# deepomicslab/PALACE

Hardware: AMD Instinct MI355X
Metric: contigs/sec eref+generate_graph+matching, 1M-contig synth, 1/2/4/8 GPU (higher is better)
Workload: dtype u32

## Files before the change

palace_amd/csrc/eref.hip:

```cpp
#include "eref_common.hpp"

namespace palace {

__global__ __launch_bounds__(256) void eref_count_kernel(const uint8_t *__restrict__ bases,
                                                         const int64_t *__restrict__ offsets,
                                                         int64_t n_reads,
                                                         const uint8_t *__restrict__ keep,
                                                         CoderMasks masks, KeyBuckets range, uint32_t *__restrict__ p1,
                                                         uint32_t *__restrict__ p2,
                                                         uint32_t *__restrict__ p3)
{
    const int lane = threadIdx.x & 63;
    const int64_t wave = (static_cast<int64_t>(blockIdx.x) * blockDim.x + threadIdx.x) >> 6;
    const int64_t n_waves = (static_cast<int64_t>(gridDim.x) * blockDim.x) >> 6;
    for (int64_t r = wave; r < n_reads; r += n_waves) {
        if (keep && !keep[r]) continue;
        const int64_t beg = offsets[r];
        const int64_t len = offsets[r + 1] - beg;
        const int64_t npos = len - 31;
        if (npos <= 0) continue;
        const uint8_t *s = bases + beg;
        Streams lo = ballot_streams(s, lane, len);
        for (int64_t base = 0; base < npos; base += 64) {
            Streams hi = ballot_streams(s, base + 64 + lane, len);
// ... 196 lines not shown
                  "the 6-position tile must fit four times into the LDS of a CU");
    __shared__ uint32_t dst[kL1Buckets];
    __shared__ uint32_t any_partial;
    const int lane = threadIdx.x & 63, wave = threadIdx.x >> 6;
#ifdef PALACE_STAMPS
    unsigned long long stamp_arr[8] = {0, 0, 0, 0, 0, 0, 0, 0};
    unsigned long long *stamps = (threadIdx.x == 0 && blockIdx.x % 7 == 0 && blockIdx.x / 7 < 65536) ? stamp_arr : nullptr;
#endif
    STAMP(stamps, 0);
    const int64_t p = pos_lo + (static_cast<int64_t>(blockIdx.x) * THREADS + threadIdx.x) * P;
    const int64_t g = min(p, pos_hi) >> 5;
    const int sh = static_cast<int>(p & 31);
    uint32_t w[2][3], uw[2];
#pragma unroll
    for (int q = 0; q < 3; q++) { w[0][q] = s0[g + q]; w[1][q] = s1[g + q]; }
    uw[0] = su[g]; uw[1] = su[g + 1];
    if (threadIdx.x < kL1Buckets) hist[threadIdx.x] = 0;
    if (threadIdx.x == kL1Buckets) any_partial = 0;
    lds_barrier();
    uint32_t u = __builtin_amdgcn_alignbit(uw[1], uw[0], sh) & ((1u << P) - 1);
    if (p >= pos_hi) u = 0;
    else if (p + P > pos_hi) u &= (1u << (pos_hi - p)) - 1;
    uint32_t key[P][3], rank[P][3];
    if (u) {
        uint32_t lo[2], hi[2];
#pragma unroll
        for (int q = 0; q < 2; q++) {
            lo[q] = __builtin_amdgcn_alignbit(w[q][1], w[q][0], sh);
            hi[q] = __builtin_amdgcn_alignbit(w[q][2], w[q][1], sh);
        }
#pragma unroll
        for (int t = 0; t < P; t++) {
            const uint32_t a0 = __builtin_amdgcn_alignbit(hi[0], lo[0], t), a1 = __builtin_amdgcn_alignbit(hi[1], lo[1], t);
            kmer_keys(masks, a0, a1, ~(a0 ^ a1), key[t]);
            if ((u >> t) & 1u) {
#pragma unroll
                for (int i = 0; i < 3; i++) {
                    const uint32_t bk = key[t][i] >> kL1Shift;
                    rank[t][i] = (!SHARE || o.keys.bucket(bk)) ? atomicAdd(&hist[bk], 1u) : ~0u;
                }
            }
        }
    }
    STAMP(stamps, 1);
    lds_barrier();
    STAMP(stamps, 2);
    const uint32_t replica = blockIdx.x % kL1Replicas;
    const bool reserver = threadIdx.x >= 64 && threadIdx.x < 64 + kL1Buckets;
    const uint32_t my_row = threadIdx.x - 64;
    uint32_t my_pc = 0, my_g = 0;
    if (wave == 0) {
        const uint32_t c0 = hist[2 * lane], c1 = hist[2 * lane + 1];
        const uint32_t pc0 = (c0 + kGroupKeys - 1) / kGroupKeys * kGroupKeys, pc1 = (c1 + kGroupKeys - 1) / kGroupKeys * kGroupKeys;
        const uint32_t incl = wave_inclusive_scan(pc0 + pc1);
        const uint32_t a0 = incl - pc0 - pc1, a1 = a0 + pc0;
        start[2 * lane] = a0; start[2 * lane + 1] = a1;
        if (lane == 63) start[kL1Buckets] = incl;
    } else if (reserver) {
        my_pc = (hist[my_row] + kGroupKeys - 1) / kGroupKeys;
        if (my_pc) my_g = atomicAdd(&o.cursor[l1_cursor(my_row, replica)], my_pc);
    }
    lds_barrier();
    STAMP(stamps, 3);
    if (u) {
#pragma unroll
        for (int t = 0; t < P; t++) {
            if ((u >> t) & 1u) {
#pragma unroll
                for (int i = 0; i < 3; i++)
                    if (!SHARE || rank[t][i] != ~0u) tile[start[key[t][i] >> kL1Shift] + rank[t][i]] = key[t][i];
            }
        }
    }
    if (reserver) {
        const uint32_t cap = o.caps.cap(my_row);
        const bool whole = static_cast<uint64_t>(my_g) + my_pc <= cap;
        room[my_row] = cap - min(cap, my_g);
        dst[my_row] = static_cast<uint32_t>(l1_region_base(o.caps, my_row, replica) + my_g - start[my_row] / kGroupKeys);
        if (!whole) any_partial = 1;
    }
    lds_barrier();
    STAMP(stamps, 4);
    const uint32_t total = start[kL1Buckets];
    const bool check = any_partial != 0;
    constexpr int kSweeps = (kMaxKeys / static_cast<int>(kGroupKeys) + THREADS - 1) / THREADS;
    uint32_t slow = 0;
    uint4 k[kSweeps];
    uint32_t to[kSweeps], live = 0;
#pragma unroll
    for (int it = 0; it < kSweeps; it++) {
        const uint32_t gi = it * THREADS + threadIdx.x, x = gi * kGroupKeys;
        to[it] = 0;
        k[it] = uint4{0, 0, 0, 0};
        if (x < total) {
            uint32_t s5[kGroupKeys];
#pragma unroll
            for (uint32_t e = 0; e < kGroupKeys; e++) s5[e] = tile[x + e];
            const uint32_t row = s5[0] >> kL1Shift;
            const uint32_t in_row = x - start[row];
            k[it] = pack_group(s5, min(kGroupKeys, hist[row] - in_row));
            if (!check || in_row / kGroupKeys < room[row]) { to[it] = dst[row] + gi; live |= 1u << it; }
            else slow |= 1u << it;
        }
    }
#pragma unroll
    for (int it = 0; it < kSweeps; it++)
        if (live & (1u << it)) reinterpret_cast<uint4 *>(o.buf)[to[it]] = k[it];
    if (slow) {
#pragma unroll 1
        for (int it = 0; it < kSweeps; it++) {
            if (!((slow >> it) & 1u)) continue;
            const uint32_t x = (it * THREADS + threadIdx.x) * kGroupKeys;
            const uint32_t row = tile[x] >> kL1Shift;
            const uint32_t n = min(kGroupKeys, hist[row] - (x - start[row]));
#pragma unroll 1
            for (uint32_t e = 0; e < n; e++) count_key_marked(tile[x + e], o.p1, o.p2, o.p3, o.touched);
        }
    }
    STAMP(stamps, 5);
#ifdef PALACE_STAMPS
    asm volatile("s_waitcnt vmcnt(0)" ::: "memory");
    STAMP(stamps, 6);
    if (stamps)
        for (int i = 0; i < 8; i++) palace_stamp_buf[(blockIdx.x / 7) * 8 + i] = stamp_arr[i];
#endif
}

__global__ __launch_bounds__(kBin2Threads) void eref_bin2_kernel(const unsigned int *__restrict__ cursor1,
                                                                 const uint32_t *__restrict__ buf1, DensityCaps caps1,
                                                                 Bin2Grid grid, Bin2Out o)
{
    __shared__ Stage2 st;
    uint32_t lo = 0, hi = kL1Buckets;
    while (hi - lo > 1) { const uint32_t mid = (lo + hi) >> 1; if (grid.first[mid] <= blockIdx.x) lo = mid; else hi = mid; }
    const uint32_t b1 = lo, within = blockIdx.x - grid.first[b1], per_region = tiles_of_bucket(caps1, b1);
    const uint32_t replica = within / per_region, tile = within % per_region;
    const uint32_t n1 = min(cursor1[l1_cursor(b1, replica)], caps1.cap(b1));
    const uint32_t start = tile * kTile2Groups;
    if (start >= n1) return;
    const uint32_t end = min(n1, start + kTile2Groups);
    const uint4 *src = reinterpret_cast<const uint4 *>(buf1) + l1_region_base(caps1, b1, replica);
    uint4 v[kGroups2PerThread];
#pragma unroll
    for (int it = 0; it < kGroups2PerThread; it++) {
        const uint32_t i = start + it * kBin2Threads + threadIdx.x;
        v[it] = i < end ? src[i] : uint4{0, 0, 0, 0};
    }
    if (threadIdx.x < kL2Rows) st.rows[threadIdx.x] = threadIdx.x * kRowSlots;
    const uint32_t cap = fine_sub_cap(o.caps, b1), xcd = xcc_id();
    __syncthreads();
    using Homeless = std::conditional_t<(kGroups2PerThread * kGroupKeys > 32), unsigned long long, uint32_t>;
    Homeless homeless = 0;
#pragma unroll
    for (int it = 0; it < kGroups2PerThread; it++) {
        uint32_t k[kGroupKeys];
        const uint32_t n = unpack_group(v[it], k);
        uint32_t at[kGroupKeys];
#pragma unroll
        for (uint32_t e = 0; e < kGroupKeys; e++) at[e] = atomicAdd(&st.rows[k[e] >> kFineBits], e < n ? 1u : 0u);
#pragma unroll
        for (uint32_t e = 0; e < kGroupKeys; e++) {
            const uint32_t row = k[e] >> kFineBits;
            const bool is_key = e < n, fits = at[e] < (row + 1) * kRowSlots;
            st.slot[is_key && fits ? at[e] : kStage2Slots] = static_cast<uint16_t>(k[e]);
            homeless |= static_cast<Homeless>(is_key && !fits ? 1u : 0u) << (kGroupKeys * it + e);
        }
    }
    if (homeless) {
#pragma unroll
        for (int it = 0; it < kGroups2PerThread; it++) {
            if (!((homeless >> (kGroupKeys * it)) & 31u)) continue;
            uint32_t k[kGroupKeys];
            unpack_group(src[start + it * kBin2Threads + threadIdx.x], k);
#pragma unroll
            for (uint32_t e = 0; e < kGroupKeys; e++) {
                if (!((homeless >> (kGroupKeys * it + e)) & 1u)) continue;
                const uint32_t row = k[e] >> kFineBits;
                const uint32_t gg = atomicAdd(&o.cursor[(b1 * kL2Rows + row) * kXcds + xcd], 1u);
                if (gg < cap) o.buf[fine_region_base(o.caps, b1, row) + static_cast<uint64_t>(xcd) * cap + gg] = static_cast<uint16_t>(k[e]);
                else count_key_marked((b1 << kL1Shift) | k[e], o.p1, o.p2, o.p3, o.touched);
            }
        }
    }
    __syncthreads();
    constexpr int rows_per_wave = kL2Rows / (kBin2Threads / 64);
    const int lane = threadIdx.x & 63;
    const int row0 = __builtin_amdgcn_readfirstlane(static_cast<int>(threadIdx.x >> 6)) * rows_per_wave;
    uint32_t c = 0, g = 0, p_lo = 0, p_hi = 0;
    bool over = false;
    if (lane < rows_per_wave) {
        const uint32_t row = row0 + lane;
        c = min(st.rows[row], (row + 1) * kRowSlots) - row * kRowSlots;
        if (c) g = atomicAdd(&o.cursor[(b1 * kL2Rows + row) * kXcds + xcd], c);
        over = static_cast<uint64_t>(g) + c > cap;
        const uint64_t ptr = reinterpret_cast<uint64_t>(o.buf + fine_region_base(o.caps, b1, row) + static_cast<uint64_t>(xcd) * cap + min(g, cap));
        p_lo = static_cast<uint32_t>(ptr); p_hi = static_cast<uint32_t>(ptr >> 32);
    }
    const unsigned long long over_rows = __ballot(over);
    const uint32_t c_fast = over ? 0u : c;
#pragma unroll
    for (int j0 = 0; j0 < rows_per_wave; j0 += 16) {
        uint16_t k[16];
#pragma unroll
        for (int j = 0; j < 16; j++) k[j] = st.slot[(row0 + j0 + j) * kRowSlots + lane];
#pragma unroll
        for (int j = 0; j < 16; j++) {
            const uint32_t cj = __builtin_amdgcn_readlane(c_fast, j0 + j);
            const uint32_t bl = __builtin_amdgcn_readlane(p_lo, j0 + j), bh = __builtin_amdgcn_readlane(p_hi, j0 + j);
            global_u16 *dst = reinterpret_cast<global_u16 *>((static_cast<uint64_t>(bh) << 32) | bl);
            if (lane < cj) dst[lane] = k[j];
        }
    }
    unsigned long long more = __ballot(lane < rows_per_wave && (c > 64 || over));
    while (more) {
        const int j = __builtin_ctzll(more);
        more &= more - 1;
        const uint32_t cj = __builtin_amdgcn_readlane(c, j);
        const uint32_t bl = __builtin_amdgcn_readlane(p_lo, j), bh = __builtin_amdgcn_readlane(p_hi, j);
        global_u16 *dst = reinterpret_cast<global_u16 *>((static_cast<uint64_t>(bh) << 32) | bl);
        const uint16_t *row_slots = st.slot + (row0 + j) * kRowSlots;
        if ((over_rows >> j) & 1ull) {
            const uint32_t gj = __builtin_amdgcn_readlane(g, j);
            const uint32_t room = cap - (gj < cap ? gj : cap);
            const uint32_t fine = b1 * kL2Rows + row0 + j;
#pragma unroll 1
            for (uint32_t q = 0; q < cj; q += 64) {
                if (q + lane < cj) {
                    const uint32_t kk = row_slots[q + lane];
                    if (q + lane < room) dst[q + lane] = static_cast<uint16_t>(kk);
                    else count_key_marked((fine << kFineBits) | kk, o.p1, o.p2, o.p3, o.touched);
                }
            }
            continue;
        }
        for (uint32_t q = 64; q < cj; q += 64)
            if (lane + q < cj) dst[lane + q] = row_slots[lane + q];
    }
}

constexpr int kCountThreads = 256;
constexpr int kProbeSetsMax = 4;
struct ProbeArgs {
    const unsigned long long *first[kProbeSetsMax];
    const uint16_t *keys16[kProbeSetsMax];
    uint8_t *ehits[kProbeSetsMax];
    const uint32_t *pos_s;
    uint8_t *sent_bytes;
};
__device__ __forceinline__ void scatter_sentinels(const ProbeArgs &pr, unsigned long long i, uint32_t m)
{
    uint32_t p[8];
#pragma unroll
    for (int e = 0; e < 8; e++) p[e] = ((m >> e) & 1u) ? pr.pos_s[i * 8 + e] : ~0u;
#pragma unroll
    for (int e = 0; e < 8; e++)
        if (p[e] != ~0u) pr.sent_bytes[p[e]] = 1;
}
__device__ __forceinline__ uint32_t count_vector(const uint32_t *__restrict__ l1, const uint32_t *__restrict__ l2, const uint32_t *__restrict__ l3, const uint4 &v)
{
    const uint32_t d[4] = {v.x, v.y, v.z, v.w};
    uint32_t m = 0;
#pragma unroll
    for (int e = 0; e < 4; e++) {
        const uint32_t k0 = d[e] & 0xffffu, k1 = d[e] >> 16;
        const uint32_t c0 = ((l1[k0 >> 5] >> (k0 & 31)) & 1u) + ((l2[k0 >> 5] >> (k0 & 31)) & 1u) + ((l3[k0 >> 5] >> (k0 & 31)) & 1u);
        const uint32_t c1 = ((l1[k1 >> 5] >> (k1 & 31)) & 1u) + ((l2[k1 >> 5] >> (k1 & 31)) & 1u) + ((l3[k1 >> 5] >> (k1 & 31)) & 1u);
        m |= c0 << (4 * e);
        m |= c1 << (4 * e + 2);
    }
    return m;
}

template <bool CLEAN, bool FINAL = false, int PROBE = 0>
__global__ __launch_bounds__(kCountThreads) void eref_lds_count_kernel(const unsigned int *__restrict__ cursor,
                                                                       const uint16_t *__restrict__ binned,
                                                                       DensityCaps caps, uint32_t *__restrict__ p1,
                                                                       uint32_t *__restrict__ p2,
                                                                       uint32_t *__restrict__ p3,
                                                                       const unsigned int *__restrict__ touched, KeyBuckets share,
                                                                       ProbeArgs pr)
{
    __shared__ uint32_t l1[kFineWords], l2[kFineWords], l3[kFineWords];
    const uint32_t b = blockIdx.x, b1 = b / kL2Rows;
    if (!share.bucket(b1)) return;
    constexpr int kProbeBatch = 2;
    unsigned long long pe0 = 0, phi = 0;
    if (PROBE) { pe0 = pr.first[0][b] / 8; phi = pr.first[0][b + 1] / 8; }
    constexpr int kLateCh = 3, kLateSent = 1;
#ifndef PALACE_PROBE_GROUP
#define PALACE_PROBE_GROUP 2
#endif
    constexpr int kProbeGroup = PALACE_PROBE_GROUP;
    constexpr bool ALL = PROBE >= 2, COUNTS = PROBE == 3;
    auto code = [&](const uint4 &vec) -> uint32_t { return COUNTS ? count_vector(l1, l2, l3, vec) : probe_vector(l3, vec); };
    auto put_code = [&](int k, unsigned long long i, uint32_t m) {
        if (COUNTS) reinterpret_cast<uint16_t *>(pr.ehits[k])[i] = static_cast<uint16_t>(m);
        else pr.ehits[k][i] = static_cast<uint8_t>(m);
    };
    unsigned long long q0[kProbeSetsMax - 1] = {0, 0, 0}, q1[kProbeSetsMax - 1] = {0, 0, 0};
    if (ALL) {
#pragma unroll
        for (int k = 1; k < kProbeSetsMax; k++) { q0[k - 1] = pr.first[k][b] / 8; q1[k - 1] = pr.first[k][b + 1] / 8; }
    }
    const uint32_t sub_cap = fine_sub_cap(caps, b1);
    uint32_t n_sub[kXcds], first[kXcds + 1];
    first[0] = 0;
#pragma unroll
    for (int x = 0; x < kXcds; x++) {
        n_sub[x] = min(cursor[b * kXcds + x], sub_cap);
        first[x + 1] = first[x] + (n_sub[x] + 7) / 8;
    }
    const uint32_t n8 = first[kXcds];
    const size_t w0 = static_cast<size_t>(b) * kFineWords;
    if (n8 == 0) {
        if (FINAL && ((touched[b >> 5] >> (b & 31)) & 1u)) {
            uint4 *z1 = reinterpret_cast<uint4 *>(p1 + w0), *z2 = reinterpret_cast<uint4 *>(p2 + w0);
            if (COUNTS) {
                for (int i = threadIdx.x; i < kFineWords / 4; i += kCountThreads) {
                    reinterpret_cast<uint4 *>(l1)[i] = z1[i];
                    reinterpret_cast<uint4 *>(l2)[i] = z2[i];
                }
            }
            for (int i = threadIdx.x; i < kFineWords / 4; i += kCountThreads) z1[i] = z2[i] = uint4{0, 0, 0, 0};
            if (ALL || (PROBE && phi > pe0)) {
                const uint4 *s3 = reinterpret_cast<const uint4 *>(p3 + w0);
                for (int i = threadIdx.x; i < kFineWords / 4; i += kCountThreads) reinterpret_cast<uint4 *>(l3)[i] = s3[i];
                __syncthreads();
                const uint4 *pv = reinterpret_cast<const uint4 *>(pr.keys16[0]);
                for (unsigned long long i = pe0 + threadIdx.x; i < phi; i += kCountThreads) put_code(0, i, code(pv[i]));
                if (ALL) {
#pragma unroll
                    for (int k = 1; k < kProbeSetsMax; k++) {
                        const uint4 *qv = reinterpret_cast<const uint4 *>(pr.keys16[k]);
                        for (unsigned long long i = q0[k - 1] + threadIdx.x; i < q1[k - 1]; i += kCountThreads) {
                            const uint32_t m = code(qv[i]);
                            if (k == 3 && !COUNTS) scatter_sentinels(pr, i, m);
                            else put_code(k, i, m);
                        }
                    }
                    uint4 *z3 = reinterpret_cast<uint4 *>(p3 + w0);
                    for (int i = threadIdx.x; i < kFineWords / 4; i += kCountThreads) z3[i] = uint4{0, 0, 0, 0};
                }
            }
        }
        return;
    }
    const uint4 *g1 = reinterpret_cast<const uint4 *>(p1 + w0), *g2 = reinterpret_cast<const uint4 *>(p2 + w0),
                *g3 = reinterpret_cast<const uint4 *>(p3 + w0);
    const uint4 *keys = reinterpret_cast<const uint4 *>(binned + fine_region_base(caps, b1, b % kL2Rows));
    auto locate = [&](uint32_t j, uint32_t &valid) -> const uint4 * {
        uint32_t x = 0, f = 0, ns = n_sub[0];
#pragma unroll
        for (int k = 1; k < kXcds; k++) {
            const uint32_t ge = j >= first[k] ? 1u : 0u;
            x += ge; f += ge * (first[k] - first[k - 1]); ns += ge * (n_sub[k] - n_sub[k - 1]);
        }
        const uint32_t local = j - f;
        valid = min(8u, ns - 8 * local);
        return keys + (static_cast<size_t>(x) * sub_cap) / 8 + local;
    };
    constexpr int kBatch = 4;
    uint4 v[kBatch];
    uint32_t ok[kBatch];
#pragma unroll
    for (int u = 0; u < kBatch; u++) {
        const uint32_t i = threadIdx.x + u * kCountThreads;
        ok[u] = 0; v[u] = uint4{0, 0, 0, 0};
        if (i < n8) v[u] = *locate(i, ok[u]);
    }
    uint4 pcur[kProbeBatch];
    if (PROBE) {
        const uint4 *pv = reinterpret_cast<const uint4 *>(pr.keys16[0]);
#pragma unroll
        for (int u = 0; u < kProbeBatch; u++) {
            const unsigned long long i = pe0 + threadIdx.x + static_cast<unsigned long long>(u) * kCountThreads;
            pcur[u] = i < phi ? pv[i] : uint4{0, 0, 0, 0};
        }
    }
    const bool seed = !CLEAN || ((touched[b >> 5] >> (b & 31)) & 1u);
    if (seed) {
        for (int i = threadIdx.x; i < kFineWords / 4; i += kCountThreads) {
            reinterpret_cast<uint4 *>(l1)[i] = g1[i];
            reinterpret_cast<uint4 *>(l2)[i] = g2[i];
            reinterpret_cast<uint4 *>(l3)[i] = g3[i];
        }
    } else {
        for (int i = threadIdx.x; i < kFineWords / 4; i += kCountThreads)
            reinterpret_cast<uint4 *>(l1)[i] = reinterpret_cast<uint4 *>(l2)[i] = reinterpret_cast<uint4 *>(l3)[i] = uint4{0, 0, 0, 0};
    }
    __syncthreads();
    auto apply = [&](uint32_t k) {
        const uint32_t w = k >> 5, bit = 1u << (k & 31);
        if (atomicOr(&l1[w], bit) & bit)
            if (atomicOr(&l2[w], bit) & bit) atomicOr(&l3[w], bit);
    };
    for (uint32_t i0 = threadIdx.x; i0 < n8; i0 += kBatch * kCountThreads) {
        uint4 nx[kBatch];
        uint32_t nok[kBatch];
#pragma unroll
        for (int u = 0; u < kBatch; u++) {
            const uint32_t i = i0 + (kBatch + u) * kCountThreads;
            nok[u] = 0; nx[u] = uint4{0, 0, 0, 0};
            if (i < n8) nx[u] = *locate(i, nok[u]);
        }
#pragma unroll
        for (int u = 0; u < kBatch; u++) {
            const uint32_t d[4] = {v[u].x, v[u].y, v[u].z, v[u].w};
#pragma unroll
            for (int e = 0; e < 4; e++) {
                if (2 * e < static_cast<int>(ok[u])) apply(d[e] & 0xffffu);
                if (2 * e + 1 < static_cast<int>(ok[u])) apply(d[e] >> 16);
            }
        }
#pragma unroll
        for (int u = 0; u < kBatch; u++) { v[u] = nx[u]; ok[u] = nok[u]; }
    }
    uint4 lch[2][kLateCh], lsn[kLateSent];
    if (ALL) {
        asm volatile("" ::: "memory");
#pragma unroll
        for (int c = 0; c < 2; c++) {
            const uint4 *qv = reinterpret_cast<const uint4 *>(pr.keys16[1 + c]);
#pragma unroll
            for (int u = 0; u < kLateCh; u++) {
                const unsigned long long i = q0[c] + threadIdx.x + static_cast<unsigned long long>(u) * kCountThreads;
                lch[c][u] = i < q1[c] ? qv[i] : uint4{0, 0, 0, 0};
            }
        }
        const uint4 *qs = reinterpret_cast<const uint4 *>(pr.keys16[3]);
#pragma unroll
        for (int u = 0; u < kLateSent; u++) {
            const unsigned long long i = q0[2] + threadIdx.x + static_cast<unsigned long long>(u) * kCountThreads;
            lsn[u] = i < q1[2] ? qs[i] : uint4{0, 0, 0, 0};
        }
    }
    __syncthreads();
    uint32_t pm[kProbeBatch], lm[2][kLateCh], sm[kLateSent];
    if (PROBE) {
#pragma unroll
        for (int u = 0; u < kProbeBatch; u++) {
            pm[u] = code(pcur[u]);
            if (ALL) asm volatile("" : "+v"(pm[u]) : : "memory");
        }
    }
    if (ALL) {
#pragma unroll
        for (int c = 0; c < 2; c++)
#pragma unroll
            for (int u = 0; u < kLateCh; u++) {
                lm[c][u] = code(lch[c][u]);
                if (COUNTS || (c * kLateCh + u) % kProbeGroup == kProbeGroup - 1) asm volatile("" : "+v"(lm[c][u]) : : "memory");
            }
#pragma unroll
        for (int u = 0; u < kLateSent; u++) { sm[u] = code(lsn[u]); asm volatile("" : "+v"(sm[u]) : : "memory"); }
    }
    if (ALL && !COUNTS) {
#pragma unroll
        for (int u = 0; u < kLateSent; u++) {
            const unsigned long long i = q0[2] + threadIdx.x + static_cast<unsigned long long>(u) * kCountThreads;
            if (i < q1[2] && sm[u]) scatter_sentinels(pr, i, sm[u]);
        }
    }
    uint4 *o1 = reinterpret_cast<uint4 *>(p1 + w0), *o2 = reinterpret_cast<uint4 *>(p2 + w0),
          *o3 = reinterpret_cast<uint4 *>(p3 + w0);
    if (ALL) {
        if (seed)
            for (int i = threadIdx.x; i < kFineWords / 4; i += kCountThreads) o1[i] = o2[i] = o3[i] = uint4{0, 0, 0, 0};
    } else {
        for (int i = threadIdx.x; i < kFineWords / 4; i += kCountThreads) {
            if (!FINAL) {
                o1[i] = reinterpret_cast<const uint4 *>(l1)[i];
                o2[i] = reinterpret_cast<const uint4 *>(l2)[i];
            } else if (seed) {
                o1[i] = o2[i] = uint4{0, 0, 0, 0};
            }
            o3[i] = reinterpret_cast<const uint4 *>(l3)[i];
        }
    }
    if (PROBE) {
#pragma unroll
        for (int u = 0; u < kProbeBatch; u++) {
            const unsigned long long i = pe0 + threadIdx.x + static_cast<unsigned long long>(u) * kCountThreads;
            if (i < phi) put_code(0, i, pm[u]);
        }
    }
    if (ALL) {
#pragma unroll
        for (int c = 0; c < 2; c++)
#pragma unroll
            for (int u = 0; u < kLateCh; u++) {
                const unsigned long long i = q0[c] + threadIdx.x + static_cast<unsigned long long>(u) * kCountThreads;
                if (i < q1[c]) put_code(1 + c, i, lm[c][u]);
            }
        if (COUNTS) {
#pragma unroll
            for (int u = 0; u < kLateSent; u++) {
                const unsigned long long i = q0[2] + threadIdx.x + static_cast<unsigned long long>(u) * kCountThreads;
                if (i < q1[2]) put_code(3, i, sm[u]);
            }
        }
    }
    if (PROBE) {
        const uint4 *pv = reinterpret_cast<const uint4 *>(pr.keys16[0]);
        for (unsigned long long i = pe0 + threadIdx.x + static_cast<unsigned long long>(kProbeBatch) * kCountThreads; i < phi; i += kCountThreads)
            put_code(0, i, code(pv[i]));
    }
    if (ALL) {
#pragma unroll
        for (int k = 1; k < kProbeSetsMax; k++) {
            const uint4 *qv = reinterpret_cast<const uint4 *>(pr.keys16[k]);
            const int held = k == 3 ? kLateSent : kLateCh;
            for (unsigned long long i = q0[k - 1] + threadIdx.x + static_cast<unsigned long long>(held) * kCountThreads; i < q1[k - 1]; i += kCountThreads) {
                const uint32_t m = code(qv[i]);
                if (k == 3 && !COUNTS) scatter_sentinels(pr, i, m);
                else put_code(k, i, m);
            }
        }
    }
}

}

using namespace palace;

static_assert(kSets == kProbeSetsMax, "the count kernel's probe arguments hold every entry set");

namespace {
int plan_count(palace_ctx *ctx, int64_t total_bases, CountPlan *pl)
{
    int64_t default_slab = 1ll << 30;
    if (ctx->slab_override == 0 && total_bases > default_slab) {
        size_t free_b = 0, total_b = 0;
        if (hipMemGetInfo(&free_b, &total_b) == hipSuccess && free_b + ctx->ws.bytes >= (160ull << 30)) default_slab = 1ll << 31;
    }
    pl->slab_bases_max = ctx->slab_override > 0 ? ctx->slab_override : default_slab;
    pl->n_slabs = (total_bases + pl->slab_bases_max - 1) / pl->slab_bases_max;
    const int64_t slab_bases = std::min(total_bases, pl->slab_bases_max);
    const int64_t max_keys = 3 * slab_bases, max_keys1 = max_keys;
    const int64_t mean1 = max_keys1 / kRegions / kGroupKeys * 26 / 25 + 1, mean2 = max_keys / kFine / 2;
    pl->caps1 = DensityCaps{static_cast<uint64_t>(mean1 + mean1 / 5), static_cast<uint32_t>(mean1 / 8 + 1024), 1};
    pl->caps2 = DensityCaps{static_cast<uint64_t>(mean2 + mean2 / 5) / 4, static_cast<uint32_t>(mean2 / 8 + 2048) / 4};
    if (ctx->bin_cap_override > 0) {
        pl->caps2 = DensityCaps{0, static_cast<uint32_t>((ctx->bin_cap_override + 3) / 4)};
        pl->caps1 = DensityCaps{0, static_cast<uint32_t>((ctx->bin_cap_override + kGroupKeys - 1) / kGroupKeys), 1};
    }
    PALACE_REQUIRE(pl->caps1.cap(0) < (1u << 31) && pl->caps2.cap(0) < (1u << 30), "slab too large for 32-bit region cursors");
    pl->cur1_bytes = align_up(kRegions * sizeof(unsigned int), 256);
    pl->cur2_bytes = align_up(static_cast<size_t>(kFine) * kXcds * sizeof(unsigned int), 256);
    pl->buf1_bytes = align_up(static_cast<size_t>(pl->caps1.prefix(kL1Buckets)) * kL1Replicas * 16, 256);
    PALACE_REQUIRE(pl->buf1_bytes < (1ull << 36), "slab too large: level 1 addresses its regions as 2^32 groups of 16 bytes");
    pl->buf2_bytes = align_up(static_cast<size_t>(pl->caps2.prefix(kL1Buckets)) * kL2Rows * 4, 256);
    pl->n_chunks = (total_bases + 63) / 64;
    pl->words_bytes = align_up(static_cast<size_t>(pl->n_chunks + 2) * 8, 256);
    PALACE_REQUIRE(pl->words_bytes >= (static_cast<size_t>(total_bases >> 5) + 3) * 4, "stream pad does not cover the last tile's look-ahead");
    PALACE_REQUIRE(pl->caps1.prefix(kL1Buckets) * kL1Replicas < (1ull << 32), "level-1 regions exceed 2^32 groups of 16 bytes");
    PALACE_REQUIRE(3ull * static_cast<uint64_t>(slab_bases) / kL1Replicas + (1ull << 20) < (1ull << 32), "slab too large for 32-bit region cursors");
    return PALACE_OK;
}
}

extern "C" {

int palace_eref_reserve(palace_ctx *ctx, int64_t total_bases)
{
    PALACE_REQUIRE(ctx && total_bases >= 0, "bad argument");
    PALACE_HIP_TRY(hipSetDevice(ctx->device));
    int rc = ensure_table(ctx);
    if (rc) return rc;
    const bool binned = ctx->probe_all_sets == 2 || ctx->count_mode == 2 || (ctx->count_mode == 0 && total_bases >= (1ll << 22));
    if (!binned) return PALACE_OK;
    CountPlan pl;
    rc = plan_count(ctx, total_bases, &pl);
    if (rc) return rc;
    return ensure_workspace(ctx, pl.total());
}

}

static int build_streams(palace_ctx *ctx, const uint8_t *d_bases, const int64_t *d_offsets, int64_t n_reads, const uint8_t *d_keep,
                         int64_t total_bases, unsigned long long *ends, unsigned long long *dropped, unsigned long long *const strm[3],
                         size_t words_bytes)
{
    const int64_t n_chunks = (total_bases + 63) / 64;
    PALACE_HIP_TRY(hipMemsetAsync(ends, 0, words_bytes, ctx->stream));
    if (d_keep) PALACE_HIP_TRY(hipMemsetAsync(dropped, 0, words_bytes, ctx->stream));
    hipLaunchKernelGGL(mark_read_ends_kernel, dim3(static_cast<unsigned>((n_reads + 255) / 256)), dim3(256), 0,
                       ctx->stream, d_offsets, n_reads, ends);
    if (d_keep)
        hipLaunchKernelGGL(mark_dropped_kernel, dim3(static_cast<unsigned>((n_reads + 255) / 256)), dim3(256), 0,
                           ctx->stream, d_offsets, n_reads, d_keep, dropped);
    PALACE_HIP_TRY(hipGetLastError());
    for (int q = 0; q < 3; q++)
        PALACE_HIP_TRY(hipMemsetAsync(strm[q] + n_chunks - 1, 0, 24, ctx->stream));
    const int64_t groups = (total_bases + 15) / 16, blocks = (groups + kStreamTile - 1) / kStreamTile;
    PALACE_REQUIRE(blocks < (1ll << 31), "too many tiles for one launch");
    hipLaunchKernelGGL(eref_streams_kernel, dim3(static_cast<unsigned>(blocks)), dim3(256), 0, ctx->stream, d_bases,
                       d_offsets, total_bases, reinterpret_cast<const uint16_t *>(ends),
                       d_keep ? reinterpret_cast<const uint16_t *>(dropped) : nullptr, reinterpret_cast<uint16_t *>(strm[0]),
                       reinterpret_cast<uint16_t *>(strm[1]), reinterpret_cast<uint16_t *>(strm[2]));
    PALACE_HIP_TRY(hipGetLastError());
    return PALACE_OK;
}

static void carve_count(const CountPlan &pl, char *ws, bool with_words, CountBufs *b)
{
    b->cursor2 = reinterpret_cast<unsigned int *>(ws); ws += pl.cur2_bytes;
    b->touched = reinterpret_cast<unsigned int *>(ws); ws += kTouchedBytes;
    b->cursor1 = reinterpret_cast<unsigned int *>(ws); ws += pl.cur1_bytes;
    if (with_words) { b->words = reinterpret_cast<unsigned long long *>(ws); ws += 5 * pl.words_bytes; }
    b->buf1 = reinterpret_cast<uint32_t *>(ws); ws += pl.buf1_bytes;
    b->buf2 = reinterpret_cast<uint16_t *>(ws);
}

static int probe_index_launch_fused(palace_ctx *ctx, const palace_eref_probe_index *ix, const CountBufs &b, const CountPlan &pl, const KeyBuckets &keys,
                                    int mode)
{
    const bool all_sets = mode >= 1;
    if (mode == 2) {
        PALACE_REQUIRE(ix->ecnt_own[0], "the probe index has no count block (palace_eref_entry_layout / _buffers_attach)");
        PALACE_REQUIRE(ix->canonical, "the probe index's entries are not in position order (a bucket of more than 8192 entries, or no room for the ordering pass): "
                                      "ranks could not add their partial counts entry by entry");
        PALACE_HIP_TRY(hipMemsetAsync(ix->ecnt_own[0], 0, 2 * ix->entry_hits_bytes, ctx->stream));
    } else if (all_sets && ix->ehits_own[0] == ix->hits_block) {
        PALACE_HIP_TRY(hipMemsetAsync(ix->hits_block, 0, ix->ehits_own_bytes, ctx->stream));
    } else {
        PALACE_HIP_TRY(hipMemsetAsync(ix->ehits_own[0], 0, all_sets ? ix->entry_hits_bytes : ix->ehits_bytes[0], ctx->stream));
        if (all_sets) PALACE_HIP_TRY(hipMemsetAsync(ix->sent_bytes_own, 0, ix->hit_bytes_size / kSentinelStride, ctx->stream));
    }
    ProbeArgs pr{};
    for (int k = 0; k < kSets; k++) {
        pr.first[k] = ix->first + static_cast<size_t>(k) * (kIndexGroups + 1);
        pr.keys16[k] = ix->keys16[k];
        pr.ehits[k] = mode == 2 ? ix->ecnt_own[k] : ix->ehits_own[k];
    }
    pr.pos_s = ix->pos_s;
    pr.sent_bytes = ix->sent_bytes_own;
    if (mode == 2)
        hipLaunchKernelGGL((eref_lds_count_kernel<true, true, 3>), dim3(kFine), dim3(kCountThreads), 0, ctx->stream, b.cursor2, b.buf2, pl.caps2,
                           ctx->plane[0], ctx->plane[1], ctx->plane[2], b.touched, keys, pr);
    else if (all_sets)
        hipLaunchKernelGGL((eref_lds_count_kernel<true, true, 2>), dim3(kFine), dim3(kCountThreads), 0, ctx->stream, b.cursor2, b.buf2, pl.caps2,
                           ctx->plane[0], ctx->plane[1], ctx->plane[2], b.touched, keys, pr);
    else
        hipLaunchKernelGGL((eref_lds_count_kernel<true, true, 1>), dim3(kFine), dim3(kCountThreads), 0, ctx->stream, b.cursor2, b.buf2, pl.caps2,
                           ctx->plane[0], ctx->plane[1], ctx->plane[2], b.touched, keys, pr);
    PALACE_HIP_TRY(hipGetLastError());
    return PALACE_OK;
}

static int partial_counts_ready(palace_ctx *ctx)
{
    const palace_eref_probe_index *ix = ctx->probe_ix;
    if (!ix || !ctx->want_final) { set_error("option probe_all_sets 2 needs option final_count and an attached probe index"); return PALACE_ESTATE; }
    if (!probe_index_usable(ctx, ix)) { set_error("probe_all_sets 2: the attached probe index was built with another coder or holds no entries"); return PALACE_ESTATE; }
    if (!ix->ecnt_own[0]) { set_error("probe_all_sets 2: the probe index has no count block (palace_eref_entry_buffers_attach)"); return PALACE_ESTATE; }
    const bool whole = (ctx->key_buckets[0] & ctx->key_buckets[1] & ctx->key_buckets[2] & ctx->key_buckets[3]) == ~0u;
    if (!whole) { set_error("probe_all_sets 2: a share of the reads is counted over the whole key space (palace_eref_set_key_buckets is set)"); return PALACE_ESTATE; }
    if (!ctx->table_clean || ctx->counts_ptr) { set_error("probe_all_sets 2: one count call per reset (the table is not clean)"); return PALACE_ESTATE; }
    return PALACE_OK;
}
static int partial_counts_zero(palace_ctx *ctx)
{
    const palace_eref_probe_index *ix = ctx->probe_ix;
    PALACE_HIP_TRY(hipSetDevice(ctx->device));
    PALACE_HIP_TRY(hipMemsetAsync(ix->ecnt_own[0], 0, 2 * ix->entry_hits_bytes, ctx->stream));
    ctx->counts_ptr = ix->ecnt_own[0];
    ctx->c0_hits_ix = nullptr;
    ctx->hits_mask = 0;
    return PALACE_OK;
}

static int launch_bin1(palace_ctx *ctx, hipStream_t stream, int ppl, const uint32_t *w0, const uint32_t *w1, const uint32_t *wu, int64_t p_lo,
                       int64_t p_hi, const BinOut &o1)
{
    const int64_t tile_pos = static_cast<int64_t>(kBinThreads) * ppl;
    const int64_t tiles = (p_hi - p_lo + tile_pos - 1) / tile_pos;
    PALACE_REQUIRE(tiles < (1ll << 31), "too many tiles for one launch");
    const dim3 grid(static_cast<unsigned>(tiles)), block(kBinThreads);
#define PALACE_BIN1(P_, SHARE_) hipLaunchKernelGGL((eref_bin1_sort_kernel<P_, kBinThreads, SHARE_>), grid, block, 0, stream, w0, w1, wu, p_lo, p_hi, ctx->masks, o1)
    if (o1.keys.all()) {
        if (ppl == 6) PALACE_BIN1(6, false); else PALACE_BIN1(8, false);
    } else {
        if (ppl == 6) PALACE_BIN1(6, true); else PALACE_BIN1(8, true);
    }
#undef PALACE_BIN1
    PALACE_HIP_TRY(hipGetLastError());
    return PALACE_OK;
}

static int bin_and_count(palace_ctx *ctx, const CountPlan &pl, const CountBufs &b, const uint32_t *w0, const uint32_t *w1,
                         const uint32_t *wu, int64_t total_bases, double keys_per_pos)
{
    ctx->c0_hits_ix = nullptr;
    const int64_t kSlabBases = pl.slab_bases_max, n_slabs = pl.n_slabs;
    const int ppl = keys_per_pos > 1.6 ? 6 : 8;
    const KeyBuckets keys = ctx_buckets(ctx);
    Bin2Grid g2;
    g2.first[0] = 0;
    for (uint32_t bk = 0; bk < kL1Buckets; bk++)
        g2.first[bk + 1] = g2.first[bk] + (keys.bucket(bk) ? tiles_of_bucket(pl.caps1, bk) * kL1Replicas : 0);
    const Bin2Out o2{b.cursor2, b.buf2, pl.caps2, ctx->plane[0], ctx->plane[1], ctx->plane[2], b.touched};
    const BinOut o1{b.cursor1, b.buf1, pl.caps1, ctx->plane[0], ctx->plane[1], ctx->plane[2], b.touched, keys};
    for (int64_t slab = 0; slab < n_slabs; slab++) {
        PALACE_HIP_TRY(hipMemsetAsync(b.cursor2, 0, pl.cur2_bytes + kTouchedBytes, ctx->stream));
        PALACE_HIP_TRY(hipMemsetAsync(b.cursor1, 0, pl.cur1_bytes, ctx->stream));
        const bool clean = ctx->table_clean && slab == 0;
        const int64_t s_lo = slab * kSlabBases, s_hi = std::min(total_bases, (slab + 1) * kSlabBases);
        int rc1 = launch_bin1(ctx, ctx->stream, ppl, w0, w1, wu, s_lo, s_hi, o1);
        if (rc1) return rc1;
        hipLaunchKernelGGL(eref_bin2_kernel, dim3(g2.first[kL1Buckets]), dim3(kBin2Threads), 0, ctx->stream, b.cursor1, b.buf1, pl.caps1, g2, o2);
        PALACE_HIP_TRY(hipGetLastError());
        const ProbeArgs no_probe{};
        if (clean && n_slabs == 1 && ctx->want_final) {
            const palace_eref_probe_index *ix = ctx->probe_ix;
            const bool whole = (ctx->key_buckets[0] & ctx->key_buckets[1] & ctx->key_buckets[2] & ctx->key_buckets[3]) == ~0u;
            if (ix && whole && probe_index_usable(ctx, ix)) {
                int rc = probe_index_launch_fused(ctx, ix, b, pl, keys, ctx->probe_all_sets);
                if (rc) return rc;
// ... 195 lines not shown
```

Measured before the change: 113.0 million.

## Assign wave-uniform key rows per XCD and peel partial tail vectors

Replaces the per-thread locate lookup over uint4 key vectors with wave-level rows of 256 full vectors per XCD sub-bucket. Address computation becomes wave-uniform and the inner apply loop loses its per-element validity checks. The partial last vector of each sub-bucket is handled separately by a few dedicated threads. Rows that are only partly filled can leave lanes idle, and the wave-per-row split may balance work less evenly when sub-buckets are small.

```diff
diff --git a/palace_amd/csrc/eref.hip b/palace_amd/csrc/eref.hip
--- a/palace_amd/csrc/eref.hip
+++ b/palace_amd/csrc/eref.hip
@@ -522,15 +522,20 @@
 #pragma unroll
         for (int k = 1; k < kProbeSetsMax; k++) { q0[k - 1] = pr.first[k][b] / 8; q1[k - 1] = pr.first[k][b + 1] / 8; }
     }
+    constexpr int kBatch = 4;
+    constexpr uint32_t kRowVecs = 64 * kBatch;
     const uint32_t sub_cap = fine_sub_cap(caps, b1);
-    uint32_t n_sub[kXcds], first[kXcds + 1];
-    first[0] = 0;
+    uint32_t n_sub[kXcds], full[kXcds], rfirst[kXcds + 1];
+    rfirst[0] = 0;
+    uint32_t n8 = 0;
 #pragma unroll
     for (int x = 0; x < kXcds; x++) {
         n_sub[x] = min(cursor[b * kXcds + x], sub_cap);
-        first[x + 1] = first[x] + (n_sub[x] + 7) / 8;
-    }
-    const uint32_t n8 = first[kXcds];
+        full[x] = n_sub[x] / 8;
+        rfirst[x + 1] = rfirst[x] + (full[x] + kRowVecs - 1) / kRowVecs;
+        n8 += (n_sub[x] + 7) / 8;
+    }
+    const uint32_t n_rows = rfirst[kXcds];
     const size_t w0 = static_cast<size_t>(b) * kFineWords;
     if (n8 == 0) {
         if (FINAL && ((touched[b >> 5] >> (b & 31)) & 1u)) {
@@ -568,25 +573,42 @@
     const uint4 *g1 = reinterpret_cast<const uint4 *>(p1 + w0), *g2 = reinterpret_cast<const uint4 *>(p2 + w0),
                 *g3 = reinterpret_cast<const uint4 *>(p3 + w0);
     const uint4 *keys = reinterpret_cast<const uint4 *>(binned + fine_region_base(caps, b1, b % kL2Rows));
-    auto locate = [&](uint32_t j, uint32_t &valid) -> const uint4 * {
-        uint32_t x = 0, f = 0, ns = n_sub[0];
+    uint32_t at_step[kXcds], till_step[kXcds];
+#pragma unroll
+    for (int k = 1; k < kXcds; k++) {
+        const uint32_t skipped = (rfirst[k] - rfirst[k - 1]) * kRowVecs;
+        at_step[k] = sub_cap / 8 - skipped;
+        till_step[k] = full[k] - full[k - 1] + skipped;
+    }
+    auto row = [&](uint32_t r, uint32_t &left) -> const uint4 * {
+        uint32_t at = 0, till = full[0];
 #pragma unroll
         for (int k = 1; k < kXcds; k++) {
-            const uint32_t ge = j >= first[k] ? 1u : 0u;
-            x += ge; f += ge * (first[k] - first[k - 1]); ns += ge * (n_sub[k] - n_sub[k - 1]);
-        }
-        const uint32_t local = j - f;
-        valid = min(8u, ns - 8 * local);
-        return keys + (static_cast<size_t>(x) * sub_cap) / 8 + local;
+            const uint32_t ge = r >= rfirst[k] ? 1u : 0u;
+            at += ge * at_step[k]; till += ge * till_step[k];
+        }
+        left = r < n_rows ? till - r * kRowVecs : 0;
+        return keys + (at + r * kRowVecs);
     };
-    constexpr int kBatch = 4;
+    constexpr uint32_t kWaves = kCountThreads / 64;
+    const uint32_t wave = __builtin_amdgcn_readfirstlane(threadIdx.x >> 6), lane = threadIdx.x & 63;
     uint4 v[kBatch];
-    uint32_t ok[kBatch];
-#pragma unroll
-    for (int u = 0; u < kBatch; u++) {
-        const uint32_t i = threadIdx.x + u * kCountThreads;
-        ok[u] = 0; v[u] = uint4{0, 0, 0, 0};
-        if (i < n8) v[u] = *locate(i, ok[u]);
+    uint32_t left;
+    {
+        const uint4 *src = row(wave, left);
+#pragma unroll
+        for (int u = 0; u < kBatch; u++)
+            if (lane + 64 * u < left) v[u] = src[lane + 64 * u];
+    }
+    uint4 tv = {0, 0, 0, 0};
+    uint32_t tn = 0;
+    if (threadIdx.x >= kCountThreads - kXcds) {
+        const uint32_t x = threadIdx.x - (kCountThreads - kXcds);
+        uint32_t ns = n_sub[0];
+#pragma unroll
+        for (int k = 1; k < kXcds; k++) ns += (x >= static_cast<uint32_t>(k) ? 1u : 0u) * (n_sub[k] - n_sub[k - 1]);
+        tn = ns & 7u;
+        if (tn) tv = keys[static_cast<size_t>(x) * (sub_cap / 8) + ns / 8];
     }
     uint4 pcur[kProbeBatch];
     if (PROBE) {
@@ -614,26 +636,32 @@
         if (atomicOr(&l1[w], bit) & bit)
             if (atomicOr(&l2[w], bit) & bit) atomicOr(&l3[w], bit);
     };
-    for (uint32_t i0 = threadIdx.x; i0 < n8; i0 += kBatch * kCountThreads) {
+    if (tn) {
+        const uint32_t d[4] = {tv.x, tv.y, tv.z, tv.w};
+#pragma unroll
+        for (int e = 0; e < 4; e++) {
+            if (2 * e < static_cast<int>(tn)) apply(d[e] & 0xffffu);
+            if (2 * e + 1 < static_cast<int>(tn)) apply(d[e] >> 16);
+        }
+    }
+    for (uint32_t r = wave; r < n_rows; r += kWaves) {
         uint4 nx[kBatch];
-        uint32_t nok[kBatch];
+        uint32_t nleft;
+        const uint4 *src = row(r + kWaves, nleft);
+#pragma unroll
+        for (int u = 0; u < kBatch; u++)
+            if (lane + 64 * u < nleft) nx[u] = src[lane + 64 * u];
 #pragma unroll
         for (int u = 0; u < kBatch; u++) {
-            const uint32_t i = i0 + (kBatch + u) * kCountThreads;
-            nok[u] = 0; nx[u] = uint4{0, 0, 0, 0};
-            if (i < n8) nx[u] = *locate(i, nok[u]);
-        }
-#pragma unroll
-        for (int u = 0; u < kBatch; u++) {
-            const uint32_t d[4] = {v[u].x, v[u].y, v[u].z, v[u].w};
-#pragma unroll
-            for (int e = 0; e < 4; e++) {
-                if (2 * e < static_cast<int>(ok[u])) apply(d[e] & 0xffffu);
-                if (2 * e + 1 < static_cast<int>(ok[u])) apply(d[e] >> 16);
-            }
-        }
-#pragma unroll
-        for (int u = 0; u < kBatch; u++) { v[u] = nx[u]; ok[u] = nok[u]; }
+            if (lane + 64 * u < left) {
+                const uint32_t d[4] = {v[u].x, v[u].y, v[u].z, v[u].w};
+#pragma unroll
+                for (int e = 0; e < 4; e++) { apply(d[e] & 0xffffu); apply(d[e] >> 16); }
+            }
+        }
+#pragma unroll
+        for (int u = 0; u < kBatch; u++) v[u] = nx[u];
+        left = nleft;
     }
     uint4 lch[2][kLateCh], lsn[kLateSent];
     if (ALL) {
```

New measurement: 113.4 million (median of 6 runs). Within noise of the previous version (+0.4%).
